# IllyaArtemchuk/Harmonies-Alphazero

Measured on AMD Instinct MI355X. Metric: self-play env-steps/sec + games/sec @4096 boards, 1/2/4/8 GPUs; bit-exact vs CPU, higher is better.
Workload: dtype u64; 1 GPU; config2: 4096 concurrent boards/GPU, reset + rule-driven play to game end (legal mask, step, chance draws, final scoring); one step = 256 hz_play launches of 4096 boards; boards_per_gpu=4096, parallelism=shard1

## Files before the change

### harmonies-alphazero_amd/csrc/hz_env.hip

```cpp
#include <hip/hip_runtime.h>

#include <cstdio>
#include <cstdlib>
#include <cstring>

#include "../../include/hz_abi.h"
#include "hz_device.hpp"
#include "hz_encode.hpp"
#include "hz_host.hpp"

using namespace hz;
using namespace hz_host;

struct P2Draw {
  int32_t *tag;
  int32_t *k;
  uint64_t *q;
  uint64_t *bag;
  int32_t *c;
};
struct P2Mid {
  int32_t *tag;
  uint64_t *st;
  uint64_t *q;
// ... 542 lines not shown
    o.get(d.tag, nr * 4);
    o.get(d.k, nr * 4);
    o.get(d.q, kAheadWords * nr * 8);
    o.get(d.bag, nr * 8);
    o.get(d.c, nr * 4);
  };
  for (int k = 0; k < kP2Draw - 1; k++) md(e->p2_x[k][0]), md(e->p2_x[k][1]);
  for (int k = 0; k < kP2Ring; k++) {
    md(e->p2_pl[k]);
    o.get(e->p2_h[k], kRulePlies * nr * 4);
    o.get(e->p2_h_tag[k], nr * 4);
  }
  for (int k = 0; k < kP2Play - 1; k++)
    for (int j = 0; j < 2; j++) {
      P2Mid &mm = e->p2_m[k][j];
      o.get(mm.tag, nr * 4);
      o.get(mm.st, 6 * nr * 8);
      o.get(mm.q, 4 * nr * 8);
      o.get(mm.i, 3 * nr * 4);
    }
  for (int k = 0; k < 2; k++) {
    o.get(e->p2_p1h[k], nr * 4);
    o.get(e->p2_p1t[k], nr * 4);
    o.get(e->p2_p2h[k], 4 * nr * 4);
    o.get(e->p2_p3h[k], 4 * nr * 4);
    o.get(e->p2_ep[k], nr * 4);
  }
  if (!o.ok || p2_clear_tags(e)) {
    o.release();
    return 1;
  }
  e->primed2 = 0;
  return 0;
}

static int launch_play2(hz_env *e, int32_t max_plies, int32_t *games_done, int32_t *steps_done) {
  if (alloc_p2(e)) return 1;
  const int c = e->calls2, r = c & 1, w = r ^ 1;
  if (!e->primed2) {
    if (hipMemcpyAsync(e->p2_ep[w], e->episode, (size_t)e->n * sizeof(int32_t), hipMemcpyDeviceToDevice,
                       e->stream))
      return 1;
    e->primed2 = 1;
  }
  P2Args a{};
  a.st = e->state;
  a.mt = e->mt;
  a.pos = e->pos;
  a.ply = e->ply;
  a.episode = e->episode;
  a.seed = e->seed;
  a.n = e->n;
  a.max_plies = max_plies;
  a.draws = e->seed_ahead;
  a.err = e->wait_err;
  a.spin = e->spin_limit;
  a.fell_lim = e->p2_fell_lim;
  for (int k = 0; k < kP2Play - 1; k++) a.cut[k] = e->p2_cut[k];
  for (int k = 0; k <= kP2Draw; k++) a.dcut[k] = e->p2_dcut[k];
  a.seed_base = e->seed_base;
  a.nrow = (long)e->nrow;
  a.games_done = games_done;
  a.steps_done = steps_done;
  a.mt_src = e->mt_src;
  a.win_tag = e->pw_tag;
  a.ep_in = e->p2_ep[w];
  a.ep_out = e->p2_ep[r];
  auto sl = [c](int s) { return ((c - s) % kP2Stream + kP2Stream) % kP2Stream; };
  for (int s = 1; s < kP2Stages; s++) {
    a.s_mt[s] = e->p2_s[sl(s)];
    a.s_tag[s] = e->p2_s_tag[sl(s)];
    a.s_cur[s] = e->p2_s_cur[sl(s)];
  }
  a.s_idx_last = sl(kP2Last);
  a.p1h_w = e->p2_p1h[r];
  a.p1h_r = e->p2_p1h[w];
  a.p1t_w = e->p2_p1t[r];
  a.p1t_r = e->p2_p1t[w];
  a.p2h_w = e->p2_p2h[r];
  a.p2h_r = e->p2_p2h[w];
  a.p3h_w = e->p2_p3h[r];
  a.p3h_r = e->p2_p3h[w];
  for (int k = 0; k < kP2Draw - 1; k++) {
    a.x_w[k] = e->p2_x[k][r];
    a.x_r[k] = e->p2_x[k][w];
  }
  a.pl_w = e->p2_pl[c % kP2Ring];
  a.h_w = e->p2_h[c % kP2Ring];
  a.ht_w = e->p2_h_tag[c % kP2Ring];
  for (int st = 0; st < kP2Play; st++) {
    const int k = (c + kP2Ring - 1 - st) % kP2Ring;
    a.pl_r[st] = e->p2_pl[k];
    a.h_r[st] = e->p2_h[k];
    a.ht_r[st] = e->p2_h_tag[k];
  }
  for (int st = 0; st < kP2Play - 1; st++) {
    a.m_w[st] = e->p2_m[st][r];
    a.m_r[st] = e->p2_m[st][w];
  }
  const int nblk = grid_for(e->n);
  hipLaunchKernelGGL(k_play2, dim3(4 * nblk), dim3(kStageThreads), kResetLds, e->stream, a, nblk);
  if (int err = launch_err()) return err;
  e->lazy = 1;
  e->calls2 = (c + 1) % (kP2Stream * kP2Ring * 2);
  e->primed = 0;
  e->ar_primed = 0;
  return 0;
}

extern "C" {

hz_env *hz_env_create(int32_t n_boards, uint64_t seed_base, void *stream) {
  if (n_boards <= 0) return nullptr;
  if (install_comp_table()) return nullptr;
  if (lds_opt_in<k_reset>(kResetLds) || lds_opt_in<k_rollout<false, false>>(kResetLds) ||
      lds_opt_in<k_rollout<false, true>>(kResetLds) || lds_opt_in<k_rollout<true, false>>(kResetLds) ||
      lds_opt_in<k_rollout<true, true>>(kResetLds) || lds_opt_in<k_play2>(kResetLds) ||
      lds_opt_in<k_mt_materialize2>(kResetLds))
    return nullptr;
  hz_env *e = new (std::nothrow) hz_env();
  if (!e) return nullptr;
  e->n = n_boards;
  e->seed_base = seed_base;
  e->stream = (hipStream_t)stream;
  const size_t n = (size_t)n_boards, nr = (n + kBlock - 1) / kBlock * kBlock, i32 = sizeof(int32_t);
  e->nrow = nr;
  DevBufs &o = e->bufs;
  o.get(e->state, n * 6 * sizeof(uint64_t), 0);
  o.get(e->mt, n * 624 * sizeof(uint32_t));
  o.get(e->pos, n * i32, 0);
  o.get(e->ply, n * i32, 0);
  o.get(e->episode, n * i32, 0);
  o.get(e->seed, n * sizeof(uint64_t), 0);
  o.get(e->mt_src, n * i32, 0xff);
  for (int k = 0; k < 2; k++) {
    o.get(e->ahead_mt[k], n * kMT * sizeof(uint32_t));
    o.get(e->ahead_tag[k], n * i32, 0xff);
    o.get(e->ahead_pile[k], n * kAheadWords * sizeof(uint64_t));
    o.get(e->ahead_cur[k], n * (kAheadDraws + 1) * i32);
    o.get(e->ahead_rule[k], nr * kRulePlies * sizeof(uint32_t));
    o.get(e->ep_final[k], n * i32);
  }
  for (int k = 0; k < kRing; k++) {
    o.get(e->ring_mt[k], nr * kMT * sizeof(uint32_t));
    o.get(e->ring_tag[k], nr * i32, 0xff);
    o.get(e->ring_pile[k], nr * 3 * sizeof(uint64_t));
    o.get(e->ring_cur[k], nr * (kD1Draws + 1) * i32);
    o.get(e->ring_k1[k], nr * i32);
  }
  o.get(e->pw_words, nr * kPlyWin * sizeof(uint32_t));
  o.get(e->pw_tag, nr * i32, 0xff);
// ... 351 lines not shown
```

### harmonies-alphazero_amd/csrc/hz_play2.hpp

```cpp
#pragma once

namespace {

#ifndef HZ_P2_ST_WT
#define HZ_P2_ST_WT 0
#endif
#ifndef HZ_P2_AUX
#define HZ_P2_AUX 16
#endif
#ifndef HZ_P2_STATIC_WIN
#define HZ_P2_STATIC_WIN 1
#endif
constexpr bool kP2StaticWin = HZ_P2_STATIC_WIN;

constexpr int kP2Win = 96;
constexpr int kP2WinRows = kP2Win + 24;
#ifndef HZ_P2_DCUT
#if HZ_P2_NDRAW == 5
#define HZ_P2_DCUT 0, 6, 11, 15, 19
#elif HZ_P2_NDRAW == 4
#define HZ_P2_DCUT 0, 7, 13, 18
#endif
#endif
constexpr int kP2DCut[kP2Draw] = {HZ_P2_DCUT};
constexpr int kP2StageDraws = 7;
#ifndef HZ_P2_PCUT
#if HZ_P2_NPLAY == 5
#define HZ_P2_PCUT 16, 32, 48, 64
#elif HZ_P2_NPLAY == 4
#define HZ_P2_PCUT 24, 40, 56
#endif
#endif
constexpr int kP2PCut[kP2Play - 1] = {HZ_P2_PCUT};
enum { kWvP1 = 8, kWvHash = 9, kWvPlay = 10, kWvIdle = 15 };
#ifndef HZ_P2_WAVES
#if HZ_P2_NDRAW == 5 && HZ_P2_NPLAY == 5
#define HZ_P2_WAVES 0, 1, 4, 9, 2, 3, 8, 10
#elif HZ_P2_NDRAW == 5
#define HZ_P2_WAVES 0, 1, 4, 9, 2, 3, 8, 15
#elif HZ_P2_NPLAY == 5
#define HZ_P2_WAVES 0, 1, 8, 9, 2, 3, 10, 15
#else
#define HZ_P2_WAVES 0, 1, 8, 9, 2, 3, 15, 15
#endif
#endif
constexpr int kP2Wave[8] = {HZ_P2_WAVES};
constexpr int p2_wave_count(int code) {
  int c = 0;
  for (int k = 0; k < 8; k++) c += kP2Wave[k] == code;
  return c;
}
constexpr bool p2_waves_ok() {
  for (int d = 0; d < 5; d++)
    if (p2_wave_count(d) != (d < kP2Draw ? 1 : 0)) return false;
  return p2_wave_count(kWvP1) == 1 && p2_wave_count(kWvHash) == 1 && p2_wave_count(kWvPlay) == (kP2Play == 5 ? 1 : 0);
}
static_assert(p2_waves_ok(), "HZ_P2_WAVES: every stage outside the seed and play blocks on exactly one wave");
constexpr int kP2MinPlies = 96;
#ifdef HZ_DIAG
constexpr int kP2Stamps = 48;
#define P2_PHASE(slot, t0)                                                                                       \
  do {                                                                                                           \
    __builtin_amdgcn_sched_barrier(0);                                                                           \
    if (g_stamps && b < a.n) g_stamps[(size_t)b * kP2Stamps + (slot)] = __builtin_amdgcn_s_memtime() - (t0); \
    __builtin_amdgcn_sched_barrier(0);                                                                           \
  } while (0)
#else
#define P2_PHASE(slot, t0) \
  do {                     \
  } while (0)
#endif
static_assert(4 * kP2WinRows * kWinStride * 4 <= (int)kResetLds, "a window per wave of a draw block");

struct P2Args {
  uint64_t *st;
  uint32_t *mt;
  int32_t *pos, *ply, *episode;
  uint64_t *seed;
  int n, max_plies, draws;
  int cut[kP2Play - 1];
  int dcut[kP2Draw + 1];
  uint64_t seed_base;
  long nrow;
  int32_t *games_done, *steps_done, *mt_src;
  int32_t *win_tag;
  const int32_t *ep_in;
  int32_t *ep_out;
  uint32_t *s_mt[kP2Stages];
  int32_t *s_tag[kP2Stages];
  int32_t *s_cur[kP2Stages];
  int s_idx_last;
  uint32_t *p1h_w;
  const uint32_t *p1h_r;
  int32_t *p1t_w;
  const int32_t *p1t_r;
  uint32_t *p2h_w;
  const uint32_t *p2h_r;
  uint32_t *p3h_w;
  const uint32_t *p3h_r;
  P2Draw x_w[kP2Draw - 1], x_r[kP2Draw - 1];
  P2Draw pl_w, pl_r[kP2Play];
  P2Mid m_w[kP2Play - 1], m_r[kP2Play - 1];
  uint32_t *h_w;
  const uint32_t *h_r[kP2Play];
  int32_t *ht_w;
  const int32_t *ht_r[kP2Play];
  int32_t *err;
  int spin;
  int fell_lim;
};

struct PlayDraw2 : PileScript {
  bool fell;
  MTR gm;
  const int32_t *cur_nd;
  __device__ __forceinline__ bool pair_pops() const { return d + 2 <= nd; }
  __device__ __forceinline__ bool lost() const { return fell && gm.over(); }
  __device__ __forceinline__ uint32_t draw_one(uint64_t misc) {
    if (d < nd) return pop();
    if (!fell) {
      gm = MTR(gm.w, gm.stride, *cur_nd, gm.lim);
      fell = true;
    }
    uint32_t p9;
    return draw_pile(misc, gm, p9) ? p9 : 0x1FFu;
  }
  __device__ __forceinline__ uint32_t operator()(uint64_t misc) { return take(misc, true); }
  __device__ __forceinline__ uint32_t take(uint64_t misc, bool want) {
    if (__all(!want || d < nd)) return pop_if(want);
    return want ? draw_one(misc) : 0x1FFu;
  }
};

template <class Draw>
__device__ __forceinline__ int p2_plies(State &s, Draw &draw, int g, int g_end, uint64_t rkey, const uint32_t *hs,
                                        size_t nr) {
  const int g0 = g;
  auto hash = [&](int ply) -> uint32_t { return hs && ply < kRulePlies ? hs[(size_t)ply * nr] : rule_h32(rkey, ply); };
  const bool all_hs = __all(hs != nullptr);
  uint32_t hn[8];
  int hn_g = -1;
  while (g < g_end) {
    if (phase_of(s.misc) == PH_OVER) break;
    if (__all(g + 8 <= g_end && turn_pair_safe(s))) {
      uint32_t h[8];
      if (__all(hn_g == g)) {
#pragma unroll
        for (int j = 0; j < 8; j++) h[j] = hn[j];
      } else if (all_hs && __all(g + 8 <= kRulePlies)) {
#pragma unroll
        for (int j = 0; j < 8; j++) h[j] = hs[(size_t)(g + j) * nr];
      } else {
#pragma unroll
        for (int j = 0; j < 8; j++) h[j] = hash(g + j);
      }
      if (all_hs && __all(g + 16 <= g_end && g + 16 <= kRulePlies)) {
#pragma unroll
        for (int j = 0; j < 8; j++) hn[j] = hs[(size_t)(g + 8 + j) * nr];
        hn_g = __builtin_amdgcn_readfirstlane(g + 8);
      }
      g += play_pair(s, draw, h);
      continue;
    }
    const int a = rule_action(s, hash(g));
    if (a < 0) break;
    step_trusted<true>(s, a, draw);
    g++;
  }
  return g - g0;
}

__device__ __forceinline__ int p2_wait(int *flag, int need, int limit, int32_t *err) {
  int v = __hip_atomic_load(flag, __ATOMIC_ACQUIRE, __HIP_MEMORY_SCOPE_WORKGROUP);
  for (int spin = 0; v < need && spin < limit; spin++) {
    __builtin_amdgcn_s_sleep(1);
    v = __hip_atomic_load(flag, __ATOMIC_ACQUIRE, __HIP_MEMORY_SCOPE_WORKGROUP);
  }
  if (v < need) {
    wait_failed(err, kWaitErrP2Twist);
    v = kMT + 1;
  }
  return v;
}
__device__ __forceinline__ void p2_publish(int *flag, int v) {
  asm volatile("" ::: "memory");
  __hip_atomic_store(flag, v, __ATOMIC_RELAXED, __HIP_MEMORY_SCOPE_WORKGROUP);
}
__device__ __forceinline__ __amdgpu_buffer_rsrc_t p2_slot_rsrc(uint32_t *slot, int b0, size_t nr) {
  const uint64_t base = (uint64_t)(slot + b0);
  uint32_t lo = __builtin_amdgcn_readfirstlane((uint32_t)base), hi = __builtin_amdgcn_readfirstlane((uint32_t)(base >> 32));
  const int bytes = __builtin_amdgcn_readfirstlane((int)((size_t)kMT * nr * 4 - (size_t)b0 * 4));
  return __builtin_amdgcn_make_buffer_rsrc((void *)(((uint64_t)hi << 32) | lo), 0, bytes, 0x00020000);
}
#ifndef HZ_P2_LDNT
#define HZ_P2_LDNT 0
#endif
__device__ __forceinline__ uint4 p2_ld4(const uint32_t *p) {
  if constexpr (HZ_P2_LDNT) {
    typedef uint32_t v4u __attribute__((ext_vector_type(4)));
    const v4u v = __builtin_nontemporal_load((const v4u *)p);
    return make_uint4(v[0], v[1], v[2], v[3]);
  }
  return *reinterpret_cast<const uint4 *>(p);
}
template <class T>
__device__ __forceinline__ void p2_st(T *p, T v) {
  if constexpr (HZ_P2_AUX == 16 && HZ_P2_ST_WT) __hip_atomic_store(p, v, __ATOMIC_RELAXED, __HIP_MEMORY_SCOPE_AGENT);
  else *p = v;
}
__device__ __forceinline__ uint32_t p1_step(uint32_t t, uint32_t q, bool odd, uint32_t kA, uint32_t kB) {
  return (t ^ ((q ^ (q >> 30)) * 1664525U)) + (odd ? kA : kB);
}
__device__ __forceinline__ uint32_t p1_row1(uint32_t kA, uint32_t kB) {
  return p1_step(kInitGen.v[1], 19650218u, true, kA, kB);
}
__device__ __forceinline__ void p2_keys(uint64_t seed, uint32_t &kA, uint32_t &kB) {
  const uint32_t key0 = (uint32_t)seed, key1 = (uint32_t)(seed >> 32);
  kA = key0;
  kB = key1 ? key1 + 1u : key0;
}

typedef uint32_t u32x8 __attribute__((ext_vector_type(8)));
template <int Imm>
__device__ __forceinline__ u32x8 p1_load8(const uint32_t *tab, uint32_t off) {
  u32x8 t;
  asm volatile("s_load_dwordx8 %0, %1, %2 offset:%3" : "=&s"(t) : "s"(tab), "s"(off), "n"(Imm));
  return t;
}
__device__ __forceinline__ void p1_arrived(u32x8 &t) { asm volatile("s_waitcnt lgkmcnt(0)" : "+s"(t)); }
__device__ __forceinline__ uint32_t p1_steps8(const u32x8 &t, uint32_t prev, uint32_t kA, uint32_t kB) {
#pragma unroll
  for (int u = 0; u < 8; u++) prev = p1_step(t[u], prev, !(u & 1), kA, kB);
  return prev;
}
__device__ __forceinline__ void p2_p1(const P2Args &a, int b) {
  const int e = a.ep_in[b] + kP2Last;
  uint32_t kA, kB;
  p2_keys(episode_seed(a.seed_base, b, e), kA, kB);
  uint32_t prev = 19650218u;
  const uint32_t *tab = kInitGen.v + 1;
  static_assert(38 * 16 + 1 == 609 && 617 + 8 <= kMT + kInitGenPad, "the last group's read (rows 617-624) within the table's padding");
  u32x8 ta = p1_load8<0>(tab, 0), tb;
  p1_arrived(ta);
#pragma unroll 1
  for (uint32_t off = 0; off < 38 * 64; off += 64) {
    tb = p1_load8<32>(tab, off);
    __builtin_amdgcn_sched_barrier(0);
    prev = p1_steps8(ta, prev, kA, kB);
    __builtin_amdgcn_sched_barrier(0);
    p1_arrived(tb);
    ta = p1_load8<64>(tab, off);
    __builtin_amdgcn_sched_barrier(0);
    prev = p1_steps8(tb, prev, kA, kB);
    __builtin_amdgcn_sched_barrier(0);
    p1_arrived(ta);
  }
  tb = p1_load8<0>(tab, (617 - 1) * 4);
// ... 80 lines not shown
  constexpr bool KeepLds = p2_mode_lds(Mode), Hbm = p2_mode_hbm(Mode);
  static_assert((G1 - G0) % 8 == 0, "groups of eight");
  static_assert(G1 + 15 < kMT + kInitGenPad, "the table's read-ahead within its padding");
  constexpr int S = kLdsStride;
  uint32_t lg = o.lds + G0 * S * 4;
#pragma unroll 2
  for (int g = G0; g < G1; g += 8) {
    uint32_t ivn[8], nx[8];
#pragma unroll
    for (int u = 0; u < 8; u++) ivn[u] = tab[g + 16 + u];
    const uint32_t kneg = __builtin_amdgcn_readfirstlane(0u - (uint32_t)g);
    [[maybe_unused]] int soff = 0;
    if constexpr (Hbm) soff = __builtin_amdgcn_readfirstlane((Mode == kP2Part ? g - 1 : g) * o.row_bytes);
    if (KeepLds) asm volatile("" : "+v"(lg));
    uint32_t q = h.cur[7];
#pragma unroll
    for (int u = 0; u < 8; u++) {
      const uint32_t p = (prev ^ (prev >> 30)) * 1566083941U;
      uint32_t v;
      asm("v_xad_u32 %0, %1, %2, %3" : "=v"(v) : "v"(p), "v"(h.cur[u]), "s"(kneg - (uint32_t)u));
      if constexpr (Hbm) o.put(Mode == kP2Part ? twist_part(prev, v) : v, soff, u);
      if (KeepLds) *(LdsWord *)(uintptr_t)(lg + u * S * 4) = v;
      prev = v;
      q = p1_step(h.iv[u], q, (G0 + u) & 1, kA, kB);
      nx[u] = q;
    }
    if (KeepLds) {
      p2_publish(prog, g + 8);
      lg += 8 * S * 4;
    }
    h.last = h.cur[7];
#pragma unroll
    for (int u = 0; u < 8; u++) {
      h.cur[u] = nx[u];
      h.iv[u] = ivn[u];
    }
  }
}
template <int G, int G1, int Mode>
__device__ __forceinline__ void p2_tail(const P2Out &o, int lane, uint32_t &prev, P2Ahead &h) {
  static_assert(G1 - G >= 1 && G1 - G <= 8, "within the group ahead");
  [[maybe_unused]] const int soff = __builtin_amdgcn_readfirstlane((Mode == kP2Part ? G - 1 : G) * o.row_bytes);
#pragma unroll
  for (int i = G; i < G1; i++) {
    const uint32_t v = (h.cur[i - G] ^ ((prev ^ (prev >> 30)) * 1566083941U)) - (uint32_t)i;
    if constexpr (p2_mode_hbm(Mode)) o.put(Mode == kP2Part ? twist_part(prev, v) : v, soff, i - G);
    if (p2_mode_lds(Mode)) hz_lds[i * kLdsStride + lane] = v;
    prev = v;
  }
  h.last = h.cur[G1 - G - 1];
}

template <int K>
__device__ __forceinline__ void p2_third(const P2Args &a, int b0, int lane, int e, bool ok, int *s_prog) {
  const int b = b0 + lane;
  const bool act = b < a.n;
  const size_t nr = (size_t)a.nrow;
  if (K == 0 && act && !ok) a.s_tag[1][b] = -1;
  if (!__any(ok)) {
    if (K == 2) p2_publish(s_prog, kMT + 1);
    return;
  }
  uint32_t *slot = a.s_mt[1 + K];
  uint32_t kA, kB;
  p2_keys(episode_seed(a.seed_base, b, e), kA, kB);
  uint32_t prev, first1, row2, q;
  if (K == 0) {
    first1 = act ? a.p1h_r[b] : 0u;
    prev = first1;
    q = p1_row1(kA, kB);
  } else {
    const uint32_t *h = K == 1 ? a.p2h_r : a.p3h_r;
    prev = act ? h[b] : 0u;
    first1 = act ? h[nr + b] : 0u;
    row2 = act ? h[2 * nr + b] : 0u;
    q = act ? h[3 * nr + b] : 0u;
  }
  const __amdgpu_buffer_rsrc_t rs = p2_slot_rsrc(slot, b0, nr);
  const int row_bytes = __builtin_amdgcn_readfirstlane((int)(nr * 4));
  const P2Out o(rs, row_bytes, lane);
  ConstWord *tab = p2_table();
  P2Ahead h;
  if constexpr (K == 0) {
    q = p1_step(kInitGen.v[2], q, false, kA, kB);
    row2 = (q ^ ((prev ^ (prev >> 30)) * 1566083941U)) - 2U;
    prev = row2;
    p2_ahead_init<3>(tab, h, q, kA, kB);
    constexpr int G = 3 + 8 * ((kP2aEnd - 3) / 8), Gp = p2_min(G, p2_up8(3, kP2PartEnd));
    p2_span<3, Gp, kP2Part>(tab, o, prev, h, kA, kB, s_prog);
    p2_span<Gp, G, kP2None>(tab, o, prev, h, kA, kB, s_prog);
    p2_tail<G, kP2aEnd, (G < kP2PartEnd ? kP2Part : kP2None)>(o, lane, prev, h);
  } else if constexpr (K == 1) {
    p2_ahead_init<kP2aEnd>(tab, h, q, kA, kB);
    constexpr int E1 = kAheadTwist + 1, Pb = p2_min(E1, p2_up8(kP2aEnd, kP2PartEnd));
    p2_span<kP2aEnd, Pb, kP2Part>(tab, o, prev, h, kA, kB, s_prog);
    p2_span<Pb, E1, kP2None>(tab, o, prev, h, kA, kB, s_prog);
    if constexpr (!HZ_P2_LEAN)
      __builtin_amdgcn_raw_buffer_store_b32(prev, rs, lane * 4, kAheadTwist * row_bytes, HZ_P2_AUX);
    p2_span<E1, kP2bDrop, kP2None>(tab, o, prev, h, kA, kB, s_prog);
    p2_span<kP2bDrop, kP2bEnd, kP2Final>(tab, o, prev, h, kA, kB, s_prog);
  } else {
    const uint32_t f0 = act ? slot[(size_t)397 * nr + b] : 0u, f1 = act ? slot[(size_t)398 * nr + b] : 0u;
    p2_ahead_init<kP2bEnd>(tab, h, q, kA, kB);
    constexpr int G = kP2bEnd + 8 * ((kMT - kP2bEnd) / 8);
    constexpr int Keep = HZ_P2_LEAN ? kP2KeepLds : kP2Keep;
    constexpr int Kc = HZ_P2_LEAN ? p2_min(G, p2_up8(kP2bEnd, kP2Twist + 397)) : G;
    p2_span<kP2bEnd, Kc, Keep>(tab, o, prev, h, kA, kB, s_prog);
    p2_span<Kc, G, kP2None>(tab, o, prev, h, kA, kB, s_prog);
    p2_tail<G, kMT, (Kc == G ? Keep : kP2None)>(o, lane, prev, h);
    p2_publish(s_prog, kMT);
    const uint32_t row1 = (first1 ^ ((prev ^ (prev >> 30)) * 1566083941U)) - 1U;
    __builtin_amdgcn_raw_buffer_store_b32(f0 ^ twist_part(0x80000000u, row1), rs, lane * 4, 0, HZ_P2_AUX);
    __builtin_amdgcn_raw_buffer_store_b32(f1 ^ twist_part(row1, row2), rs, lane * 4, row_bytes, HZ_P2_AUX);
  }
  if (K < 2) {
    if (ok) {
      uint32_t *ho = K == 0 ? a.p2h_w : a.p3h_w;
      ho[b] = prev;
      ho[nr + b] = first1;
      ho[2 * nr + b] = row2;
      ho[3 * nr + b] = h.last;
      a.s_tag[1 + K][b] = e * 8 + 3 + K;
    }
  } else if (ok) {
    a.s_tag[3][b] = e * 8 + 5;
  }
}

#ifndef HZ_P2_TWGO
// ... 7 lines not shown
}
__device__ __forceinline__ void p2_twist(const P2Args &a, int b0, int lane, bool any, int *s_prog) {
  if (!any) return;
  const size_t nr = (size_t)a.nrow;
  uint32_t *slot = a.s_mt[3];
  const int grp = lane >> 4, c4 = (lane & 15) * 4;
  uint32_t *col = slot + b0 + c4;
  auto row = [&](int r) { return p2_ld4(col + (size_t)r * nr); };
  const __amdgpu_buffer_rsrc_t rs = p2_slot_rsrc(slot, b0, nr);
  const int row_bytes = __builtin_amdgcn_readfirstlane((int)(nr * 4));
  auto store = [&](int r, const uint4 &v) {
    typedef uint32_t v4u __attribute__((ext_vector_type(4)));
    __builtin_amdgcn_raw_buffer_store_b128(v4u{v.x, v.y, v.z, v.w}, rs, c4 * 4 + r * row_bytes, 0, HZ_P2_AUX);
  };
  [[maybe_unused]] const int b = b0 + lane;
  HZ_DIAG_T0(tz);
  int have = kTwGo >= 0 ? p2_wait(s_prog, kP2bEnd + kTwGo, a.spin, a.err) : 0;
  P2_PHASE(35, tz);
  uint4 pt[kTwIters], fh[kTwHbm];
#pragma unroll
  for (int i = 0; i < kTwIters; i++) {
    const int r = grp + 4 * i;
    pt[i] = r >= 2 ? row(r) : make_uint4(0, 0, 0, 0);
  }
#pragma unroll
  for (int i = 0; i < kTwHbm; i++) {
    const int r = grp + 4 * i + 397;
    fh[i] = r < kP2bEnd ? row(r) : make_uint4(0, 0, 0, 0);
  }
  auto far = [&](int i) -> uint4 {
    const int r = grp + 4 * i;
    if (i < kTwHbm && r + 397 < kP2bEnd) return fh[i < kTwHbm ? i : 0];
    const uint32_t *d = hz_lds + (r + 397) * kLdsStride + c4;
    return make_uint4(d[0], d[1], d[2], d[3]);
  };
#pragma unroll
  for (int i = 0; i < kTwIters; i += 2) {
    const int need = 4 * (i + 1) + 3 + 397 + 1;
    if (need > kP2bEnd && have < need) have = p2_wait(s_prog, need, a.spin, a.err);
    const uint4 f0 = far(i), f1 = far(i + 1);
    if (i > 0 || grp >= 2) store(grp + 4 * i, xor4(f0, pt[i]));
    store(grp + 4 * (i + 1), xor4(f1, pt[i + 1]));
    if (i == 0) P2_PHASE(36, tz);
  }
  P2_PHASE(37, tz);
}

__device__ __forceinline__ void p2_seed(const P2Args &a, int blk) {
  __shared__ int s_prog;
  const int tid = threadIdx.x, lane = tid & 63, w = tid >> 6;
  const int b0 = blk * kBlock, b = b0 + lane;
  const bool act = b < a.n;
  if (tid == 0) s_prog = 0;
  const int k = w < 3 ? w : 2;
  const int e = act ? a.ep_in[b] + kP2Last - 1 - k : 0;
  const bool ok = act && (k == 0 ? a.p1t_r[b] : a.s_tag[1 + k][b]) == e * 8 + 2 + k;
  __syncthreads();
  if (w == 0) p2_third<0>(a, b0, lane, e, ok, &s_prog);
  else if (w == 1) p2_third<1>(a, b0, lane, e, ok, &s_prog);
  else if (w == 2) p2_third<2>(a, b0, lane, e, ok, &s_prog);
  else p2_twist(a, b0, lane, __any(ok), &s_prog);
}

__device__ __forceinline__ int wave_min_i(int v) {
#pragma unroll
  for (int o = 32; o > 0; o >>= 1) v = min(v, __shfl_xor(v, o));
  return v;
}
__device__ __forceinline__ void p2_draw_stage(const P2Args &a, int b0, int lane, int stage, int base) {
  const int b = b0 + lane;
  HZ_DIAG_T0(t0);
  const bool act = b < a.n;
  const size_t nr = (size_t)a.nrow;
  const int d0 = a.dcut[stage], d1 = stage == kP2Draw - 1 ? a.draws : min(a.draws, a.dcut[stage + 1]);
  const int e = act ? a.ep_in[b] + kP2Last - kP2SDraw - stage : 0;
  const uint32_t *slot = a.s_mt[kP2SDraw + stage];
  int32_t *cur = a.s_cur[kP2SDraw + stage] + b;
  const P2Draw &in = a.x_r[stage > 0 ? stage - 1 : 0];
  const P2Draw &out = stage == kP2Draw - 1 ? a.pl_w : a.x_w[stage < kP2Draw - 1 ? stage : 0];
  bool ok = act && a.s_tag[kP2SDraw + stage][b] == e * 8 + 5;
  int k0 = 0, c0 = kP2Ahead;
  uint64_t bag = initial_bag(), q[kAheadWords] = {0, 0, 0, 0};
  constexpr int U = kP2Win / 4;
  const int c4 = (lane & 15) * 4;
  uint4 v[U];
  auto win_load = [&](int r0) {
#pragma unroll
    for (int u = 0; u < U; u++) {
      const int r = r0 + 4 * u + (lane >> 4);
      v[u] = p2_ld4(slot + (size_t)r * nr + b0 + c4);
    }
  };
  auto win_store = [&]() {
#pragma unroll
    for (int u = 0; u < U; u++)
      *reinterpret_cast<uint4 *>(hz_lds + base + (4 * u + (lane >> 4)) * kWinStride + c4) = v[u];
  };
  const int rs = kP2StaticWin ? __builtin_amdgcn_readfirstlane((3 * d0) & ~3) : 0;
  if (kP2StaticWin || stage == 0) win_load(rs);
  if (stage > 0 && act) {
    const int itag = in.tag[b];
    k0 = in.k[b];
    c0 = in.c[b];
    bag = in.bag[b];
#pragma unroll
    for (int i = 0; i < kAheadWords; i++) q[i] = in.q[(size_t)i * nr + b];
    ok = ok && itag == e * 8 + stage;
  }
  bool draws = ok && k0 >= d0 && d0 < d1;
  int r0 = rs;
  if constexpr (kP2StaticWin) {
    draws = draws && (c0 & 0xFFFF) >= r0;
    win_store();
  } else {
    r0 = wave_min_i(draws ? (c0 & 0xFFFF) : kP2Twist) & ~3;
    if (r0 < kP2Twist) {
      if (stage > 0) win_load(r0);
      win_store();
    }
  }
  P2_PHASE(28 + stage, t0);
  if (!act) return;
  if (!ok) {
    out.tag[b] = -1;
    return;
  }
  if (stage == 0) cur[0] = kP2Ahead;
  int k = k0, cc = c0;
  if (draws) {
    const int lim = min(r0 + kP2Win, kP2Twist);
    StreamDraw<WinMT> d{WinMT(base - r0 * kWinStride + lane, c0, lim)};
#pragma unroll 1
    for (int i = d0; i < d1; i++) {
      if (d.m.pos >= lim) break;
      const uint32_t p9 = d(bag);
      if (d.m.pos > lim) break;
      apply_pile_fast(bag, p9);
      const int bit = 9 * i, wd = bit >> 6, off = bit & 63;
      const uint64_t lo9 = (uint64_t)p9 << off, hi9 = off > 55 ? (uint64_t)p9 >> (64 - off) : 0ull;
      q[0] |= wd == 0 ? lo9 : 0ull;
      q[1] |= wd == 1 ? lo9 : wd == 0 ? hi9 : 0ull;
      q[2] |= wd == 2 ? lo9 : wd == 1 ? hi9 : 0ull;
      q[3] |= wd == 3 ? lo9 : wd == 2 ? hi9 : 0ull;
      cc = d.m.cursor();
      p2_st(&cur[(size_t)(i + 1) * nr], cc);
      k = i + 1;
    }
  }
  p2_st(&out.k[b], k);
  p2_st(&out.c[b], cc);
  p2_st(&out.bag[b], bag);
#pragma unroll
  for (int i = 0; i < kAheadWords; i++) p2_st(&out.q[(size_t)i * nr + b], q[i]);
  p2_st(&out.tag[b], e * 8 + stage + 1);
}

__device__ __forceinline__ void p2_hashes(const P2Args &a, int b) {
  const size_t nr = (size_t)a.nrow;
  const int e = a.ep_in[b] + kP2Last - (kP2SPlay - 1);
  const uint64_t rk = rule_key(episode_seed(a.seed_base, b, e));
#pragma unroll 1
  for (int j = 0; j < kRulePlies; j++) p2_st(&a.h_w[(size_t)j * nr + b], rule_h32(rk, j));
  a.ht_w[b] = e;
}

__device__ __forceinline__ void p2_draw(const P2Args &a, int blk, int code) {
  const int tid = threadIdx.x, lane = tid & 63, w = tid >> 6;
  const int b0 = blk * kBlock;
  if (code < kP2Draw) {
    p2_draw_stage(a, b0, lane, code, w * kP2WinRows * kWinStride);
  } else if (code == kWvP1 && b0 + lane < a.n) {
    p2_p1(a, b0 + lane);
  } else if (code == kWvHash && b0 + lane < a.n) {
    p2_hashes(a, b0 + lane);
  }
}

__device__ __forceinline__ void p2_mid_put(const P2Mid &m, size_t nr, int b, const State &s, const PlayDraw2 &d, int g,
                                           int e) {
#pragma unroll
  for (int k = 0; k < 4; k++) p2_st(&m.st[(size_t)k * nr + b], s.pl[k]);
  p2_st(&m.st[4 * nr + b], s.piles);
  p2_st(&m.st[5 * nr + b], s.misc);
  p2_st(&m.q[b], d.q0);
  p2_st(&m.q[nr + b], d.q1);
  p2_st(&m.q[2 * nr + b], d.q2);
  p2_st(&m.q[3 * nr + b], d.q3);
  p2_st(&m.i[b], d.d);
  p2_st(&m.i[nr + b], g);
  p2_st(&m.i[2 * nr + b], d.fell ? d.gm.cursor() : -1);
  p2_st(&m.tag[b], e);
}
__device__ __forceinline__ PlayDraw2 p2_mid_get(const P2Mid &m, size_t nr, int b, State &s, int &g, int nd,
                                               uint32_t *slot, const int32_t *cur, int fell_lim) {
#pragma unroll
  for (int k = 0; k < 4; k++) s.pl[k] = m.st[(size_t)k * nr + b];
  s.piles = m.st[4 * nr + b];
  s.misc = m.st[5 * nr + b];
  const int d = m.i[b], fc = m.i[2 * nr + b];
  g = m.i[nr + b];
  return PlayDraw2{{m.q[b], m.q[nr + b], m.q[2 * nr + b], m.q[3 * nr + b], d, nd}, fc >= 0,
                   MTR(slot, (int)nr, fc >= 0 ? fc : 0, fell_lim), cur + (size_t)nd * nr};
}

__device__ __forceinline__ void p2_play(const P2Args &a, int blk, int st, bool in_block) {
  __shared__ uint64_t s_lds_mask;
  const int tid = threadIdx.x, lane = tid & 63, w = tid >> 6;
  const int b0 = blk * kBlock, b = b0 + lane;
  const bool act = b < a.n;
  const uint64_t actmask = __ballot(act);
  const int nb = a.n - b0 < kBlock ? a.n - b0 : kBlock;
  const size_t nr = (size_t)a.nrow;
  HZ_DIAG_T0(t0);
  const bool last = st == kP2Play - 1;
  bool lds_used = false;
  if (act) {
    const int e = last ? a.episode[b] : a.ep_in[b] + kP2Play - 1 - st;
    const P2Draw &pl = a.pl_r[st];
    const uint32_t *hsrc = a.h_r[st];
    const int32_t *htag = a.ht_r[st];
    uint32_t *slot = a.s_mt[kP2SPlay + st] + b;
    const int32_t *cur = a.s_cur[kP2SPlay + st] + b;
    const int g_end = last ? a.max_plies : min(a.cut[st < kP2Play - 1 ? st : 0], a.max_plies);
    const uint64_t sd = episode_seed(a.seed_base, b, e), rk = rule_key(sd);
    const int ptag = pl.tag[b], nd = pl.k[b];
    const int mtag = st > 0 ? a.m_r[st - 1].tag[b] : e;
    const uint32_t *hs = htag[b] == e ? hsrc + b : nullptr;
    State s;
    int g = 0;
    PlayDraw2 draw = st == 0 ? PlayDraw2{{pl.q[b], pl.q[nr + b], pl.q[2 * nr + b], pl.q[3 * nr + b], 0, nd}, false,
                                         MTR(slot, (int)nr, 0, a.fell_lim), cur + (size_t)nd * nr}
                             : p2_mid_get(a.m_r[st - 1], nr, b, s, g, nd, slot, cur, a.fell_lim);
    bool prep = ptag == e * 8 + kP2Draw && mtag == e;
    if (prep) {
      if (st == 0) {
        if (__all(nd >= 5)) draw.scripted_reset(s);
        else reset_state(s, draw);
      }
      P2_PHASE(16 + 2 * st, t0);
      g += p2_plies(s, draw, g, g_end, rk, hs, nr);
      P2_PHASE(17 + 2 * st, t0);
      if (draw.lost()) prep = false;
    }
    if (!last) {
      const P2Mid &mo = a.m_w[st < kP2Play - 1 ? st : 0];
      if (prep) p2_mid_put(mo, nr, b, s, draw, g, e);
      else mo.tag[b] = -1;
    } else {
      int cursor, src;
      if (prep) {
        cursor = draw.fell ? draw.gm.cursor() : cur[(size_t)draw.d * nr];
        src = 2 + a.s_idx_last;
      } else {
        mt_seed(hz_lds + lane, kLdsStride, sd);
        PlayDraw fb{{0, 0, 0, 0, 0, 0}, LdsMT(lane, kMTSeeded), false, false, MT(nullptr, 0), nullptr};
        reset_state(s, fb);
        g = p2_plies(s, fb, 0, a.max_plies, rk, nullptr, nr);
        cursor = fb.m.cursor();
        src = -1;
        lds_used = true;
      }
      a.episode[b] = e + 1;
      if (score_pending(s.misc)) finish_game(s);
      P2_PHASE(27, t0);
      store_state(a.st, a.n, b, s);
      a.pos[b] = cursor;
      a.mt_src[b] = src;
      a.win_tag[b] = -1;
      a.ply[b] = g;
      a.seed[b] = sd;
      a.ep_out[b] = e + 1;
      if (a.games_done) a.games_done[b] = phase_of(s.misc) == PH_OVER ? 1 : 0;
      if (a.steps_done) a.steps_done[b] = g;
    }
    if (in_block) P2_PHASE(w, t0);
  }
  if (!in_block) return;
  if (w == 0) {
    const uint64_t lm = __ballot(lds_used);
    if (lane == 0) s_lds_mask = lm;
  }
  __syncthreads();
  const uint64_t lds_mask = s_lds_mask & actmask;
  if (lds_mask) stage_mt(a.mt + (size_t)b0 * kMT, nb, tid, lds_mask, false);
}

__global__ void __launch_bounds__(kStageThreads) __attribute__((amdgpu_waves_per_eu(1, 1))) k_play2(P2Args a, int nblk) {
  const int blk = (int)blockIdx.x;
  const int role = blk / nblk;
  const int rb = blk - role * nblk;
  const int wv = __builtin_amdgcn_readfirstlane((int)(threadIdx.x >> 6));
  const int code = role == 1 || role == 2 ? kP2Wave[4 * (role - 1) + wv] : kWvIdle;
  const int st = role == 0 ? kP2Play - 1 - wv : code == kWvPlay ? 0 : -1;
#ifdef HZ_DIAG
  if (g_role_only >= 0 && g_role_only != role) return;
  const uint64_t t0 = __builtin_amdgcn_s_memtime(), r0 = __builtin_amdgcn_s_memrealtime();
#endif
  if (st >= 0) p2_play(a, rb, st, role == 0);
// ... 47 lines not shown
```

Baseline: 23.85 billion env-steps/s.

## Precompute per-stage kernel args on host and hoist all per-board input loads

The host now builds per-stage argument structs for the draw and play stages, resolving ring indices, cut points and draw ranges ahead of time. Each stage loads these into scalar registers through asm constraints. All of a board's global inputs (episode, tags, queue words, mid-state, first eight rule hashes) are then issued together at stage entry with clamped indices and 32-bit offsets. The aim is to overlap load latency and cut redundant address arithmetic. The cost is higher register pressure from the many loads in flight and a larger kernel argument block.

```diff
diff --git a/harmonies-alphazero_amd/csrc/hz_env.hip b/harmonies-alphazero_amd/csrc/hz_env.hip
--- a/harmonies-alphazero_amd/csrc/hz_env.hip
+++ b/harmonies-alphazero_amd/csrc/hz_env.hip
@@ -618,12 +618,8 @@
   a.seed = e->seed;
   a.n = e->n;
   a.max_plies = max_plies;
-  a.draws = e->seed_ahead;
   a.err = e->wait_err;
   a.spin = e->spin_limit;
-  a.fell_lim = e->p2_fell_lim;
-  for (int k = 0; k < kP2Play - 1; k++) a.cut[k] = e->p2_cut[k];
-  for (int k = 0; k <= kP2Draw; k++) a.dcut[k] = e->p2_dcut[k];
   a.seed_base = e->seed_base;
   a.nrow = (long)e->nrow;
   a.games_done = games_done;
@@ -633,36 +629,54 @@
   a.ep_in = e->p2_ep[w];
   a.ep_out = e->p2_ep[r];
   auto sl = [c](int s) { return ((c - s) % kP2Stream + kP2Stream) % kP2Stream; };
-  for (int s = 1; s < kP2Stages; s++) {
+  for (int s = 1; s < kP2SDraw; s++) {
     a.s_mt[s] = e->p2_s[sl(s)];
     a.s_tag[s] = e->p2_s_tag[sl(s)];
-    a.s_cur[s] = e->p2_s_cur[sl(s)];
   }
   a.s_idx_last = sl(kP2Last);
   a.p1h_w = e->p2_p1h[r];
-  a.p1h_r = e->p2_p1h[w];
   a.p1t_w = e->p2_p1t[r];
-  a.p1t_r = e->p2_p1t[w];
   a.p2h_w = e->p2_p2h[r];
-  a.p2h_r = e->p2_p2h[w];
   a.p3h_w = e->p2_p3h[r];
-  a.p3h_r = e->p2_p3h[w];
-  for (int k = 0; k < kP2Draw - 1; k++) {
-    a.x_w[k] = e->p2_x[k][r];
-    a.x_r[k] = e->p2_x[k][w];
-  }
-  a.pl_w = e->p2_pl[c % kP2Ring];
+  a.seed_tag[0] = e->p2_p1t[w];
+  a.seed_tag[1] = a.s_tag[2];
+  a.seed_tag[2] = a.s_tag[3];
+  a.seed_h[0] = e->p2_p1h[w];
+  a.seed_h[1] = e->p2_p2h[w];
+  a.seed_h[2] = e->p2_p3h[w];
+  const int draws = e->seed_ahead;
+  for (int k = 0; k < kP2Draw; k++) {
+    P2DrawArgs &d = a.dr[k];
+    const int s = kP2SDraw + k;
+    d.slot = e->p2_s[sl(s)];
+    d.stag = e->p2_s_tag[sl(s)];
+    d.cur = e->p2_s_cur[sl(s)];
+    d.in = e->p2_x[k > 0 ? k - 1 : 0][w];
+    d.out = k == kP2Draw - 1 ? e->p2_pl[c % kP2Ring] : e->p2_x[k][r];
+    d.d0 = e->p2_dcut[k];
+    d.d1 = k == kP2Draw - 1 ? draws : std::min(draws, e->p2_dcut[k + 1]);
+  }
   a.h_w = e->p2_h[c % kP2Ring];
   a.ht_w = e->p2_h_tag[c % kP2Ring];
   for (int st = 0; st < kP2Play; st++) {
+    P2PlayArgs &p = a.pp[st];
+    const bool last = st == kP2Play - 1;
+    const int s = kP2SPlay + st;
     const int k = (c + kP2Ring - 1 - st) % kP2Ring;
-    a.pl_r[st] = e->p2_pl[k];
-    a.h_r[st] = e->p2_h[k];
-    a.ht_r[st] = e->p2_h_tag[k];
-  }
-  for (int st = 0; st < kP2Play - 1; st++) {
-    a.m_w[st] = e->p2_m[st][r];
-    a.m_r[st] = e->p2_m[st][w];
+    p.ep = last ? e->episode : e->p2_ep[w];
+    p.ep_off = last ? 0 : kP2Play - 1 - st;
+    p.g0 = st > 0 ? e->p2_cut[st - 1] : 0;
+    p.g_end = last ? max_plies : std::min(e->p2_cut[st], max_plies);
+    p.fell_lim = e->p2_fell_lim;
+    p.ptag = e->p2_pl[k].tag;
+    p.pk = e->p2_pl[k].k;
+    p.q = st > 0 ? e->p2_m[st - 1][w].q : e->p2_pl[k].q;
+    p.h = e->p2_h[k];
+    p.ht = e->p2_h_tag[k];
+    p.slot = e->p2_s[sl(s)];
+    p.cur = e->p2_s_cur[sl(s)];
+    p.in = e->p2_m[st > 0 ? st - 1 : 0][w];
+    p.out = e->p2_m[last ? 0 : st][r];
   }
   const int nblk = grid_for(e->n);
   hipLaunchKernelGGL(k_play2, dim3(4 * nblk), dim3(kStageThreads), kResetLds, e->stream, a, nblk);
diff --git a/harmonies-alphazero_amd/csrc/hz_play2.hpp b/harmonies-alphazero_amd/csrc/hz_play2.hpp
--- a/harmonies-alphazero_amd/csrc/hz_play2.hpp
+++ b/harmonies-alphazero_amd/csrc/hz_play2.hpp
@@ -65,49 +65,69 @@
     if (g_stamps && b < a.n) g_stamps[(size_t)b * kP2Stamps + (slot)] = __builtin_amdgcn_s_memtime() - (t0); \
     __builtin_amdgcn_sched_barrier(0);                                                                           \
   } while (0)
+#define P2_USE_V(x) asm volatile("" ::"v"(x))
+#define P2_USE_S(x) asm volatile("" ::"s"(x))
 #else
 #define P2_PHASE(slot, t0) \
   do {                     \
   } while (0)
+#define P2_USE_V(x) \
+  do {              \
+  } while (0)
+#define P2_USE_S(x) \
+  do {              \
+  } while (0)
 #endif
 static_assert(4 * kP2WinRows * kWinStride * 4 <= (int)kResetLds, "a window per wave of a draw block");
 
+struct P2DrawArgs {
+  const uint32_t *slot;
+  const int32_t *stag;
+  int32_t *cur;
+  P2Draw in, out;
+  int d0, d1;
+};
+struct P2PlayArgs {
+  const int32_t *ep;
+  int ep_off;
+  int g0;
+  int g_end;
+  int fell_lim;
+  const int32_t *ptag, *pk;
+  const uint64_t *q;
+  const uint32_t *h;
+  const int32_t *ht;
+  uint32_t *slot;
+  const int32_t *cur;
+  P2Mid in, out;
+};
 struct P2Args {
   uint64_t *st;
   uint32_t *mt;
   int32_t *pos, *ply, *episode;
   uint64_t *seed;
-  int n, max_plies, draws;
-  int cut[kP2Play - 1];
-  int dcut[kP2Draw + 1];
+  int n, max_plies;
   uint64_t seed_base;
   long nrow;
   int32_t *games_done, *steps_done, *mt_src;
   int32_t *win_tag;
   const int32_t *ep_in;
   int32_t *ep_out;
-  uint32_t *s_mt[kP2Stages];
-  int32_t *s_tag[kP2Stages];
-  int32_t *s_cur[kP2Stages];
+  P2DrawArgs dr[kP2Draw];
+  P2PlayArgs pp[kP2Play];
+  uint32_t *s_mt[kP2SDraw];
+  int32_t *s_tag[kP2SDraw];
+  const int32_t *seed_tag[3];
+  const uint32_t *seed_h[3];
   int s_idx_last;
   uint32_t *p1h_w;
-  const uint32_t *p1h_r;
   int32_t *p1t_w;
-  const int32_t *p1t_r;
   uint32_t *p2h_w;
-  const uint32_t *p2h_r;
   uint32_t *p3h_w;
-  const uint32_t *p3h_r;
-  P2Draw x_w[kP2Draw - 1], x_r[kP2Draw - 1];
-  P2Draw pl_w, pl_r[kP2Play];
-  P2Mid m_w[kP2Play - 1], m_r[kP2Play - 1];
   uint32_t *h_w;
-  const uint32_t *h_r[kP2Play];
   int32_t *ht_w;
-  const int32_t *ht_r[kP2Play];
   int32_t *err;
   int spin;
-  int fell_lim;
 };
 
 struct PlayDraw2 : PileScript {
@@ -134,12 +154,17 @@
 
 template <class Draw>
 __device__ __forceinline__ int p2_plies(State &s, Draw &draw, int g, int g_end, uint64_t rkey, const uint32_t *hs,
-                                        size_t nr) {
+                                        size_t nr, const uint32_t *h0 = nullptr, int h0_g = -1) {
   const int g0 = g;
   auto hash = [&](int ply) -> uint32_t { return hs && ply < kRulePlies ? hs[(size_t)ply * nr] : rule_h32(rkey, ply); };
   const bool all_hs = __all(hs != nullptr);
   uint32_t hn[8];
   int hn_g = -1;
+  if (h0 && all_hs) {
+#pragma unroll
+    for (int j = 0; j < 8; j++) hn[j] = h0[j];
+    hn_g = h0_g;
+  }
   while (g < g_end) {
     if (phase_of(s.misc) == PH_OVER) break;
     if (__all(g + 8 <= g_end && turn_pair_safe(s))) {
@@ -203,6 +228,20 @@
   }
   return *reinterpret_cast<const uint4 *>(p);
 }
+template <class T>
+__device__ __forceinline__ T p2_at(const T *base, uint32_t off) {
+  typedef __attribute__((address_space(1))) const char GlobalByte;
+  typedef __attribute__((address_space(1))) const T GlobalT;
+  return *(GlobalT *)((GlobalByte *)base + off);
+}
+template <class T>
+__device__ __forceinline__ const T *p2_row(const T *base, size_t row_words) {
+  const T *p = base + row_words;
+  asm volatile("" : "+s"(p));
+  return p;
+}
+__device__ __forceinline__ void p2_fence() { asm volatile("" ::: "memory"); }
+__device__ __forceinline__ void p2_fence_use(int &x) { asm volatile("" : "+v"(x)::"memory"); }
 template <class T>
 __device__ __forceinline__ void p2_st(T *p, T v) {
   if constexpr (HZ_P2_AUX == 16 && HZ_P2_ST_WT) __hip_atomic_store(p, v, __ATOMIC_RELAXED, __HIP_MEMORY_SCOPE_AGENT);
@@ -389,7 +428,8 @@
 }
 
 template <int K>
-__device__ __forceinline__ void p2_third(const P2Args &a, int b0, int lane, int e, bool ok, int *s_prog) {
+__device__ __forceinline__ void p2_third(const P2Args &a, int b0, int lane, int e, bool ok, const uint32_t (&hw)[4],
+                                         int *s_prog) {
   const int b = b0 + lane;
   const bool act = b < a.n;
   const size_t nr = (size_t)a.nrow;
@@ -403,15 +443,14 @@
   p2_keys(episode_seed(a.seed_base, b, e), kA, kB);
   uint32_t prev, first1, row2, q;
   if (K == 0) {
-    first1 = act ? a.p1h_r[b] : 0u;
+    first1 = act ? hw[0] : 0u;
     prev = first1;
     q = p1_row1(kA, kB);
   } else {
-    const uint32_t *h = K == 1 ? a.p2h_r : a.p3h_r;
-    prev = act ? h[b] : 0u;
-    first1 = act ? h[nr + b] : 0u;
-    row2 = act ? h[2 * nr + b] : 0u;
-    q = act ? h[3 * nr + b] : 0u;
+    prev = act ? hw[0] : 0u;
+    first1 = act ? hw[1] : 0u;
+    row2 = act ? hw[2] : 0u;
+    q = act ? hw[3] : 0u;
   }
   const __amdgpu_buffer_rsrc_t rs = p2_slot_rsrc(slot, b0, nr);
   const int row_bytes = __builtin_amdgcn_readfirstlane((int)(nr * 4));
@@ -525,16 +564,60 @@
   const int b0 = blk * kBlock, b = b0 + lane;
   const bool act = b < a.n;
   if (tid == 0) s_prog = 0;
-  const int k = w < 3 ? w : 2;
-  const int e = act ? a.ep_in[b] + kP2Last - 1 - k : 0;
-  const bool ok = act && (k == 0 ? a.p1t_r[b] : a.s_tag[1 + k][b]) == e * 8 + 2 + k;
+  const int wv = __builtin_amdgcn_readfirstlane(w);
+  const int k = wv < 3 ? wv : 2;
+  const int32_t *tagp = a.seed_tag[k];
+  const uint32_t *hp = a.seed_h[k];
+  const int32_t *ep_in = a.ep_in;
+  const int n = a.n;
+  const size_t hrow = k == 0 ? 0 : (size_t)a.nrow;
+  asm volatile("" ::"s"(tagp), "s"(hp), "s"(ep_in), "s"(n), "s"(hrow));
+  __builtin_amdgcn_sched_barrier(0);
+  const int bc = min(b, n - 1);
+  const int hb = wv < 3 ? bc : b0;
+  const uint32_t *hrp[4];
+#pragma unroll
+  for (int i = 0; i < 4; i++) hrp[i] = p2_row(hp, i * hrow);
+  p2_fence();
+  int ep = p2_at(ep_in, (uint32_t)bc * 4u);
+  const int tag = p2_at(tagp, (uint32_t)bc * 4u);
+  uint32_t hw[4];
+#pragma unroll
+  for (int i = 0; i < 4; i++) hw[i] = p2_at(hrp[i], (uint32_t)hb * 4u);
+  p2_fence_use(ep);
+  const int e = act ? ep + kP2Last - 1 - k : 0;
+  const bool ok = act && tag == e * 8 + 2 + k;
   __syncthreads();
-  if (w == 0) p2_third<0>(a, b0, lane, e, ok, &s_prog);
-  else if (w == 1) p2_third<1>(a, b0, lane, e, ok, &s_prog);
-  else if (w == 2) p2_third<2>(a, b0, lane, e, ok, &s_prog);
+  if (w == 0) p2_third<0>(a, b0, lane, e, ok, hw, &s_prog);
+  else if (w == 1) p2_third<1>(a, b0, lane, e, ok, hw, &s_prog);
+  else if (w == 2) p2_third<2>(a, b0, lane, e, ok, hw, &s_prog);
   else p2_twist(a, b0, lane, __any(ok), &s_prog);
 }
 
+__device__ __forceinline__ P2DrawArgs p2_draw_args(const P2Args &a, int stage, int &n, size_t &nr,
+                                                   const int32_t *&ep_in) {
+  const P2DrawArgs r = a.dr[stage];
+  n = a.n;
+  nr = (size_t)a.nrow;
+  ep_in = a.ep_in;
+  asm volatile("" ::"s"(r.slot), "s"(r.stag), "s"(r.cur), "s"(r.in.tag), "s"(r.in.k), "s"(r.in.q), "s"(r.in.bag),
+               "s"(r.in.c), "s"(r.out.tag), "s"(r.out.k), "s"(r.out.q), "s"(r.out.bag), "s"(r.out.c), "s"(r.d0),
+               "s"(r.d1), "s"(n), "s"(nr), "s"(ep_in));
+  __builtin_amdgcn_sched_barrier(0);
+  return r;
+}
+__device__ __forceinline__ P2PlayArgs p2_play_args(const P2Args &a, int st, int &n, size_t &nr, uint64_t &seed_base) {
+  const P2PlayArgs r = a.pp[st];
+  n = a.n;
+  nr = (size_t)a.nrow;
+  seed_base = a.seed_base;
+  asm volatile("" ::"s"(r.ep), "s"(r.ep_off), "s"(r.g0), "s"(r.g_end), "s"(r.ptag), "s"(r.pk), "s"(r.q), "s"(r.h),
+               "s"(r.ht), "s"(r.slot), "s"(r.cur), "s"(r.in.tag), "s"(r.in.st), "s"(r.in.q), "s"(r.in.i),
+               "s"(r.out.tag), "s"(r.out.st), "s"(r.out.q), "s"(r.out.i), "s"(n), "s"(nr), "s"(seed_base),
+               "s"(r.fell_lim));
+  __builtin_amdgcn_sched_barrier(0);
+  return r;
+}
 __device__ __forceinline__ int wave_min_i(int v) {
 #pragma unroll
   for (int o = 32; o > 0; o >>= 1) v = min(v, __shfl_xor(v, o));
@@ -543,15 +626,16 @@
 __device__ __forceinline__ void p2_draw_stage(const P2Args &a, int b0, int lane, int stage, int base) {
   const int b = b0 + lane;
   HZ_DIAG_T0(t0);
-  const bool act = b < a.n;
-  const size_t nr = (size_t)a.nrow;
-  const int d0 = a.dcut[stage], d1 = stage == kP2Draw - 1 ? a.draws : min(a.draws, a.dcut[stage + 1]);
-  const int e = act ? a.ep_in[b] + kP2Last - kP2SDraw - stage : 0;
-  const uint32_t *slot = a.s_mt[kP2SDraw + stage];
-  int32_t *cur = a.s_cur[kP2SDraw + stage] + b;
-  const P2Draw &in = a.x_r[stage > 0 ? stage - 1 : 0];
-  const P2Draw &out = stage == kP2Draw - 1 ? a.pl_w : a.x_w[stage < kP2Draw - 1 ? stage : 0];
-  bool ok = act && a.s_tag[kP2SDraw + stage][b] == e * 8 + 5;
+  int n;
+  size_t nr;
+  const int32_t *ep_in;
+  const P2DrawArgs r = p2_draw_args(a, stage, n, nr, ep_in);
+  if (stage == 1) P2_PHASE(33, t0);
+  const int d0 = r.d0, d1 = r.d1;
+  const bool act = b < n;
+  const uint32_t *slot = r.slot;
+  int32_t *cur = r.cur + b;
+  const P2Draw &in = r.in, &out = r.out;
   int k0 = 0, c0 = kP2Ahead;
   uint64_t bag = initial_bag(), q[kAheadWords] = {0, 0, 0, 0};
   constexpr int U = kP2Win / 4;
@@ -570,15 +654,39 @@
       *reinterpret_cast<uint4 *>(hz_lds + base + (4 * u + (lane >> 4)) * kWinStride + c4) = v[u];
   };
   const int rs = kP2StaticWin ? __builtin_amdgcn_readfirstlane((3 * d0) & ~3) : 0;
+  const int bc = min(b, n - 1), bi = stage > 0 ? bc : b0;
+  const uint32_t o4 = (uint32_t)bc * 4u, i4 = (uint32_t)bi * 4u, i8 = i4 * 2u;
+  const uint64_t *iqr[kAheadWords];
+#pragma unroll
+  for (int i = 0; i < kAheadWords; i++) iqr[i] = p2_row(in.q, (size_t)i * nr);
+  p2_fence();
+  int ep = p2_at(ep_in, o4);
+  const int stag = p2_at(r.stag, o4);
+  const int itag = p2_at(in.tag, i4), ik = p2_at(in.k, i4), ic = p2_at(in.c, i4);
+  const uint64_t ibag = p2_at(in.bag, i8);
+  uint64_t iq[kAheadWords];
+#pragma unroll
+  for (int i = 0; i < kAheadWords; i++) iq[i] = p2_at(iqr[i], i8);
+  p2_fence();
   if (kP2StaticWin || stage == 0) win_load(rs);
-  if (stage > 0 && act) {
-    const int itag = in.tag[b];
-    k0 = in.k[b];
-    c0 = in.c[b];
-    bag = in.bag[b];
-#pragma unroll
-    for (int i = 0; i < kAheadWords; i++) q[i] = in.q[(size_t)i * nr + b];
+  p2_fence_use(ep);
+  if (stage == 1) {
+    P2_USE_V(ep);
+    P2_PHASE(34, t0);
+  }
+  const int e = act ? ep + kP2Last - kP2SDraw - stage : 0;
+  bool ok = act && stag == e * 8 + 5;
+  if (stage > 0) {
+    k0 = ik;
+    c0 = ic;
+    bag = ibag;
+#pragma unroll
+    for (int i = 0; i < kAheadWords; i++) q[i] = iq[i];
     ok = ok && itag == e * 8 + stage;
+  }
+  if (stage == 1) {
+    P2_USE_V((int)ok);
+    P2_PHASE(26, t0);
   }
   bool draws = ok && k0 >= d0 && d0 < d1;
   int r0 = rs;
@@ -664,59 +772,94 @@
   p2_st(&m.i[2 * nr + b], d.fell ? d.gm.cursor() : -1);
   p2_st(&m.tag[b], e);
 }
-__device__ __forceinline__ PlayDraw2 p2_mid_get(const P2Mid &m, size_t nr, int b, State &s, int &g, int nd,
-                                               uint32_t *slot, const int32_t *cur, int fell_lim) {
-#pragma unroll
-  for (int k = 0; k < 4; k++) s.pl[k] = m.st[(size_t)k * nr + b];
-  s.piles = m.st[4 * nr + b];
-  s.misc = m.st[5 * nr + b];
-  const int d = m.i[b], fc = m.i[2 * nr + b];
-  g = m.i[nr + b];
-  return PlayDraw2{{m.q[b], m.q[nr + b], m.q[2 * nr + b], m.q[3 * nr + b], d, nd}, fc >= 0,
-                   MTR(slot, (int)nr, fc >= 0 ? fc : 0, fell_lim), cur + (size_t)nd * nr};
-}
 
 __device__ __forceinline__ void p2_play(const P2Args &a, int blk, int st, bool in_block) {
   __shared__ uint64_t s_lds_mask;
   const int tid = threadIdx.x, lane = tid & 63, w = tid >> 6;
   const int b0 = blk * kBlock, b = b0 + lane;
-  const bool act = b < a.n;
-  const uint64_t actmask = __ballot(act);
-  const int nb = a.n - b0 < kBlock ? a.n - b0 : kBlock;
-  const size_t nr = (size_t)a.nrow;
   HZ_DIAG_T0(t0);
   const bool last = st == kP2Play - 1;
+  int n;
+  size_t nr;
+  uint64_t seed_base;
+  const P2PlayArgs r = p2_play_args(a, st, n, nr, seed_base);
+  const int fell_lim = r.fell_lim;
+  if (last) P2_PHASE(38, t0);
+  const bool act = b < n;
+  const uint64_t actmask = __ballot(act);
+  const int nb = n - b0 < kBlock ? n - b0 : kBlock;
+  const int bc = min(b, n - 1), bi = st > 0 ? bc : b0;
+  const uint32_t c4 = (uint32_t)bc * 4u, c8 = c4 * 2u, i4 = (uint32_t)bi * 4u, i8 = i4 * 2u;
+  const bool h0_fits = r.g0 + 8 <= kRulePlies;
+  const int h0_g = h0_fits ? r.g0 : -1;
+  const size_t h0_row = h0_fits ? (size_t)r.g0 : 0;
+  const uint64_t *qr[4], *str[6];
+  const int32_t *ir[3];
+  const uint32_t *hr[8];
+#pragma unroll
+  for (int k = 0; k < 4; k++) qr[k] = p2_row(r.q, (size_t)k * nr);
+#pragma unroll
+  for (int k = 0; k < 6; k++) str[k] = p2_row(r.in.st, (size_t)k * nr);
+#pragma unroll
+  for (int k = 0; k < 3; k++) ir[k] = p2_row(r.in.i, (size_t)k * nr);
+#pragma unroll
+  for (int j = 0; j < 8; j++) hr[j] = p2_row(r.h, (h0_row + j) * nr);
+  p2_fence();
+  int ep = p2_at(r.ep, c4);
+  const int ptag = p2_at(r.ptag, c4), nd = p2_at(r.pk, c4), itag = p2_at(r.in.tag, i4), htg = p2_at(r.ht, c4);
+  const int id = p2_at(ir[0], i4), ig = p2_at(ir[1], i4), ifc = p2_at(ir[2], i4);
+  uint64_t sq[4], ist[6];
+#pragma unroll
+  for (int k = 0; k < 4; k++) sq[k] = p2_at(qr[k], c8);
+#pragma unroll
+  for (int k = 0; k < 6; k++) ist[k] = p2_at(str[k], i8);
+  uint32_t h0[8];
+#pragma unroll
+  for (int j = 0; j < 8; j++) h0[j] = p2_at(hr[j], c4);
+  p2_fence_use(ep);
+  if (last) {
+    P2_USE_V(ep);
+    P2_PHASE(39, t0);
+  }
   bool lds_used = false;
   if (act) {
-    const int e = last ? a.episode[b] : a.ep_in[b] + kP2Play - 1 - st;
-    const P2Draw &pl = a.pl_r[st];
-    const uint32_t *hsrc = a.h_r[st];
-    const int32_t *htag = a.ht_r[st];
-    uint32_t *slot = a.s_mt[kP2SPlay + st] + b;
-    const int32_t *cur = a.s_cur[kP2SPlay + st] + b;
-    const int g_end = last ? a.max_plies : min(a.cut[st < kP2Play - 1 ? st : 0], a.max_plies);
-    const uint64_t sd = episode_seed(a.seed_base, b, e), rk = rule_key(sd);
-    const int ptag = pl.tag[b], nd = pl.k[b];
-    const int mtag = st > 0 ? a.m_r[st - 1].tag[b] : e;
-    const uint32_t *hs = htag[b] == e ? hsrc + b : nullptr;
+    const int e = ep + r.ep_off;
+    const P2Mid &mo = r.out;
+    uint32_t *slot = r.slot + b;
+    const int32_t *cur = r.cur + b;
+    const int g_end = r.g_end;
+    const uint64_t sd = episode_seed(seed_base, b, e), rk = rule_key(sd);
+    const int mtag = st > 0 ? itag : e;
+    const uint32_t *hs = htg == e ? r.h + b : nullptr;
     State s;
     int g = 0;
-    PlayDraw2 draw = st == 0 ? PlayDraw2{{pl.q[b], pl.q[nr + b], pl.q[2 * nr + b], pl.q[3 * nr + b], 0, nd}, false,
-                                         MTR(slot, (int)nr, 0, a.fell_lim), cur + (size_t)nd * nr}
-                             : p2_mid_get(a.m_r[st - 1], nr, b, s, g, nd, slot, cur, a.fell_lim);
+    PlayDraw2 draw{{sq[0], sq[1], sq[2], sq[3], 0, nd}, false, MTR(slot, (int)nr, 0, fell_lim), cur + (size_t)nd * nr};
+    if (st > 0) {
+#pragma unroll
+      for (int k = 0; k < 4; k++) s.pl[k] = ist[k];
+      s.piles = ist[4];
+      s.misc = ist[5];
+      g = ig;
+      draw.d = id;
+      draw.fell = ifc >= 0;
+      draw.gm = MTR(slot, (int)nr, ifc >= 0 ? ifc : 0, fell_lim);
+    }
     bool prep = ptag == e * 8 + kP2Draw && mtag == e;
+    if (last) {
+      P2_USE_V((int)prep);
+      P2_PHASE(42, t0);
+    }
     if (prep) {
       if (st == 0) {
         if (__all(nd >= 5)) draw.scripted_reset(s);
         else reset_state(s, draw);
       }
       P2_PHASE(16 + 2 * st, t0);
-      g += p2_plies(s, draw, g, g_end, rk, hs, nr);
+      g += p2_plies(s, draw, g, g_end, rk, hs, nr, h0, h0_g);
       P2_PHASE(17 + 2 * st, t0);
       if (draw.lost()) prep = false;
     }
     if (!last) {
-      const P2Mid &mo = a.m_w[st < kP2Play - 1 ? st : 0];
       if (prep) p2_mid_put(mo, nr, b, s, draw, g, e);
       else mo.tag[b] = -1;
     } else {
```

After: 24.86 billion env-steps/s (median of 6 runs). 1.04x the previous value.
